# kouyt5/lightning-asr

Hardware: AMD Instinct MI355X
Metric: audio-seconds/sec training (asr13x1, bs=32, 10 s clips) (higher is better)
Workload: dtype bf16; 1 GPU; asr13x1 QuartzNet-CTC train step, bs=32/GPU, 10 s synthetic 16 kHz clips, labels.txt vocab (C=28), HIP mel+conv+CTC+NovoGrad, random-init weights; global_batch=32, n_class=28, parallelism=dp1, feature_prefetch=True, hip_graph=True, staged_backward=False

## Files before the change

### include/lasr.h

```cpp
#ifndef LASR_H
#define LASR_H

#include <stddef.h>
#include <stdint.h>

#ifdef __cplusplus
extern "C" {
#endif

#define LASR_VERSION 108

enum { LASR_F32 = 0, LASR_BF16 = 1 };
enum { LASR_ACT_NONE = 0, LASR_ACT_RELU = 1, LASR_ACT_SWISH = 2 };
enum { LASR_VARIANT_PLAIN = 0, LASR_VARIANT_CONTEXT = 1, LASR_VARIANT_CONTEXT_SE = 2 };
enum {
  LASR_E_ARG = -1,
  LASR_E_SHAPE = -2,
  LASR_E_WORKSPACE = -3,
  LASR_E_FORMAT = -4,
  LASR_E_UNSUPPORTED = -5,
  LASR_E_IO = -6
};

int lasr_version(void);
// ... 75 lines not shown
int lasr_bn_finalize(const float* stats, const float* gamma, const float* beta, float* running_mean,
                     float* running_var, float* coef, float* saved, int64_t C, int64_t n_rows, float eps,
                     float momentum, int training, void* stream);
typedef struct {
  const float* gamma; const float* beta; const float* running_mean; const float* running_var; float* coef; int64_t C;
} lasr_bn_eval_desc;
int lasr_bn_eval_coef_many(const lasr_bn_eval_desc* descs, int n_descs, float eps, void* stream);

typedef struct {
  const float* partials; int n_partials;
  const float* gamma; const float* beta; float* running_mean; float* running_var;
  float* coef; float* saved; float* stats;
} lasr_bn_branch;
int lasr_bn_finalize_partials(const lasr_bn_branch* branches, int n_branches, int64_t C, int64_t n_rows, float eps,
                              float momentum, void* stream);

typedef struct { const uint64_t* step; uint64_t seed; uint32_t unit; float p; } lasr_dropout;
int lasr_mask_lengths_step(const float* pct, int64_t B, int64_t T, int32_t* lens, uint64_t* step_counter, void* stream);
int lasr_dropout_mask(const lasr_dropout* dropout, int64_t n, uint8_t* keep, void* stream);
int lasr_bn_act_fwd_drop(const void* y, const float* coef, const void* y2, const float* coef2, const float* se_scale, void* out,
                         int dtype, int64_t B, int64_t T, int64_t C, int act, const lasr_dropout* dropout, void* stream);
int lasr_bn_act_bwd_stats_drop(const void* dout, const void* y, const float* coef, const float* saved, const void* y2,
                               const float* coef2, const float* saved2, const float* se_scale, const float* se_grad, float* sums,
                               float* sums2, int dtype, int64_t B, int64_t T, int64_t C, int act, const lasr_dropout* dropout,
                               void* workspace, size_t workspace_bytes, void* stream);
int lasr_se_bwd_drop(const void* dout, const void* y, const float* coef, const void* y2, const float* coef2, const float* scale,
                     const float* hidden, const float* pooled, const float* W1, const float* W2, int dtype, int64_t B, int64_t T,
                     int64_t C, int act, const lasr_dropout* dropout, float* seg, float* dW1, float* dW2, void* workspace,
                     size_t workspace_bytes, void* stream);
size_t lasr_bn_se_bwd_workspace_bytes(int64_t B, int64_t T, int64_t C);
// ... 248 lines not shown
```

### lightning_asr_amd/_lib.py

```python
from __future__ import annotations

import ctypes as C
import os

_HERE = os.path.dirname(os.path.abspath(__file__))
LIB_PATH = os.environ.get("LASR_LIB_PATH", os.path.join(_HERE, "liblasr.so"))

F32, BF16 = 0, 1
ACT_NONE, ACT_RELU, ACT_SWISH = 0, 1, 2
LEN_LEAD = 1 << 30
VARIANT = {"plain": 0, "context": 1, "context_se": 2}

_p, _i64, _i32, _f32, _sz = C.c_void_p, C.c_int64, C.c_int, C.c_float, C.c_size_t


class Dropout(C.Structure):
    _fields_ = [("step", C.c_void_p), ("seed", C.c_uint64), ("unit", C.c_uint32), ("p", C.c_float)]


class WaveSrc(C.Structure):
    _fields_ = [("wave", C.c_void_p), ("wave_dtype", C.c_int32), ("dither", C.c_void_p), ("dither_seed", C.c_uint64),
                ("dither_step", C.c_void_p), ("pitch", C.c_int64)]


# ... 29 lines not shown
    "lasr_gemm_batch": (_i32, [_p, _i32, _i32, _i32, _i32, _i32, _i32, _p, _sz, _p]),
    "lasr_bn_finalize": (_i32, [_p, _p, _p, _p, _p, _p, _p, _i64, _i64, _f32, _f32, _i32, _p]),
    "lasr_bn_eval_coef_many": (_i32, [_p, _i32, _f32, _p]),
    "lasr_bn_act_fwd": (_i32, [_p, _p, _p, _p, _p, _p, _i32, _i64, _i64, _i64, _i32, _p]),
    "lasr_bn_bwd_workspace_bytes": (_sz, [_i64, _i64, _i64]),
    "lasr_bn_act_bwd_stats": (_i32, [_p] * 11 + [_i32, _i64, _i64, _i64, _i32, _p, _sz, _p]),
    "lasr_bn_act_bwd_apply": (_i32, [_p] * 20 + [_i32, _i64, _i64, _i64, _i32, _p, _sz, _p]),
    "lasr_bn_bwd_apply_workspace_bytes": (_sz, [_i64]),
    "lasr_reduce_many": (_i32, [_p, _i32, _p]),
    "lasr_gemm_batch_split_partials": (_i32, [_p, _i32, _i32, _i32, _i32, _i32, _p, _sz, _p, _p, _p]),
    "lasr_gemm_multi_split_partials": (_i32, [_p, _i32, _i32, _p, _p, _p]),
    "lasr_dwconv_wgrad_partials": (_i32, [_p, _p, _i32, _i64, _i64, _i64, _i32, _i32, _p, _sz, _p, _p]),
    "lasr_dwconv_bwd_fused": (_i32, [_p, _p, _p, _p, _p, _i32, _i64, _i64, _i64, _i32, _p, _sz, _p, _p]),
    "lasr_gemm_batch_partials": (_i32, [_p, _i32, _i32, _i32, _i32, _i32, _p, _sz, _p, _p, _p]),
    "lasr_bn_finalize_partials": (_i32, [_p, _i32, _i64, _i64, C.c_float, C.c_float, _p]),
    "lasr_seqsum": (_i32, [_p, _i32, _i64, _i64, _i64, _p, _p]),
    "lasr_se_fwd": (_i32, [_p, _p, _p, _p, _i64, _i64, _i64, _p, _p, _p, _p]),
    "lasr_se_bwd_workspace_bytes": (_sz, [_i64, _i64]),
    "lasr_se_bwd": (_i32, [_p] * 10 + [_i32, _i64, _i64, _i64, _i32, _p, _p, _p, _p, _sz, _p]),
    "lasr_bilstm_saved_bytes": (_sz, [_i64, _i64]),
    "lasr_bilstm_fwd": (_i32, [_p] * 9 + [_i64, _i64, _p, _i32, _i64, _i64, _p, _p]),
    "lasr_bilstm_bwd_workspace_bytes": (_sz, [_i64]),
    "lasr_bilstm_bwd": (_i32, [_p, _i32, _i64, _i64, _p, _p, _p, _i64, _i64, _p, _p, _p, _p, _p, _p, _sz, _p]),
    "lasr_copy_cols": (_i32, [_p, _i32, _i64, _i64, _p, _i32, _i64, _i64, _i64, _i64, _i32, _p]),
    "lasr_log_softmax": (_i32, [_p, _p, _p, _i64, _i64, _p]),
    "lasr_log_softmax_bwd": (_i32, [_p, _p, _p, _i64, _i64, _p]),
    "lasr_ctc_workspace_bytes": (_sz, [_i64, _i64, _i64]),
    "lasr_ctc_loss": (_i32, [_p, _p, _p, _p, _i64, _i64, _i64, _i64, _i32, _p, _p, _p, _p, _sz, _p]),
    "lasr_ctc_loss_mel": (_i32, [_p, _p, _p, _p, _i64, _i64, _i64, _i64, _i32, _p, _p, _p, _p, _sz,
                                 _p, _p, _p, _p, _i64, _i64, _i32, _p, _p, _i32, _p, _p, _p, _sz, _p]),
# ... 126 lines not shown
```

### lightning_asr_amd/csrc/conv.hip

```cpp
#include "common.h"
#include "fused.h"

namespace lasr {

static thread_local const DwTapCtx* g_dw_tap_ctx = nullptr;
void dw_taps_set_ctx(const DwTapCtx* ctx) { g_dw_tap_ctx = ctx; }
bool dw_taps_enabled() {
  static const bool on = !(getenv("LASR_DW_TAPS") && atoi(getenv("LASR_DW_TAPS")) == 0);
  return on;
}
const uint32_t* dw_taps_for(const float* w, int flip, int64_t C) {
  (void)flip;
  const DwTapCtx* c = g_dw_tap_ctx;
  if (!c || C % 64 != 0) return nullptr;
  for (int i = 0; i < c->n; ++i)
    if (c->w[i] == w && c->C[i] == (int)C) return c->t[i];
  return nullptr;
}

static constexpr int kCB = 64;
static constexpr int kTT = 128;
static constexpr int kR = 8;
static constexpr int kMaxK = 128;

// ... 422 lines not shown
namespace dwm {
static constexpr int TT = 512;
static constexpr int KWMAX = 128;
static constexpr int TIN = TT - 16 + KWMAX;
static constexpr int LDI = 1296;
static constexpr int RS = 128;
static constexpr int LDST = 160;
static constexpr int IMG_BYTES = kCB * LDI;
static constexpr int STAGE_BYTES = RS * LDST;
static constexpr int WROW = 160;
static constexpr int WSM_OFF = IMG_BYTES + STAGE_BYTES;
static constexpr int SMEM = WSM_OFF + kCB * WROW * 4;
static_assert(LDI >= TIN * 2 && LDI % 16 == 0, "image pitch");
}
struct DwBnIn {
  const bf16_t* y; const bf16_t* y2; const float* coef; const float* coef2; bf16_t* out; int act;
};
typedef __bf16 dw_bf16x8 __attribute__((ext_vector_type(8)));
typedef float dw_f32x4 __attribute__((ext_vector_type(4)));
typedef short dw_s16x4 __attribute__((ext_vector_type(4)));

#ifdef LASR_DW_STAMPS
__device__ unsigned long long* g_dw_stamps = nullptr;
#define DW_STAMP(i_) do { if (g_dw_stamps && threadIdx.x == 0) g_dw_stamps[(blockIdx.y * gridDim.x + blockIdx.x) * 8 + (i_)] = wall_clock64(); } while (0)
#else
#define DW_STAMP(i_) do {} while (0)
#endif
template <int NKS, int NSET, bool FUSE = false>
__device__ __forceinline__ void dwconv_s1_mfma_body(const bf16_t* __restrict__ x, const float* __restrict__ w,
                                                    const bf16_t* __restrict__ addend, bf16_t* __restrict__ y,
                                                    int Tlen, int C, int k, int flip, int bx, int by, int bz, int gz,
                                                    char* smem_raw, const uint32_t* __restrict__ taps, const DwBnIn bn = DwBnIn{}) {
  using namespace dwm;
  char* img = smem_raw;
  char* stage = smem_raw + IMG_BYTES;
  uint32_t* wsm = reinterpret_cast<uint32_t*>(smem_raw + WSM_OFF);
  const int tid = threadIdx.x, lane = tid & 63, wid = tid >> 6;
  const int b = by, c0 = bx * kCB;
  if (taps) {
    static_assert(WROW == kDwTapRow, "tap table row");
    const uint4* src = reinterpret_cast<const uint4*>(taps + ((size_t)flip * C + c0) * WROW);
    uint4 tv[kCB * WROW / 4 / 512];
#pragma unroll
    for (int it = 0; it < kCB * WROW / 4 / 512; ++it) tv[it] = src[tid + 512 * it];
#pragma unroll
    for (int it = 0; it < kCB * WROW / 4 / 512; ++it) reinterpret_cast<uint4*>(wsm)[tid + 512 * it] = tv[it];
  } else {
    constexpr int kIt = kCB * WROW / 512;
    float f0[kIt], f1[kIt];
#pragma unroll
    for (int it = 0; it < kIt; ++it) {
      const int i = tid + 512 * it;
      const int ch = i / WROW, idx = i - ch * WROW;
      const int i0 = idx < 80 ? 2 * idx : 2 * (idx - 80) + 1;
      const int j0 = i0 - 24, j1 = i0 - 23;
      const float* wc = w + (size_t)min(c0 + ch, C - 1) * k;
      const bool cok = c0 + ch < C;
      const int q0 = min(max(j0, 0), k - 1), q1 = min(max(j1, 0), k - 1);
      const float a0 = wc[flip ? k - 1 - q0 : q0], a1 = wc[flip ? k - 1 - q1 : q1];
      f0[it] = __uint_as_float(__float_as_uint(a0) & ((cok && j0 >= 0 && j0 < k) ? 0xffffffffu : 0u));
      f1[it] = __uint_as_float(__float_as_uint(a1) & ((cok && j1 >= 0 && j1 < k) ? 0xffffffffu : 0u));
    }
    __builtin_amdgcn_sched_barrier(0);
#pragma unroll
    for (int it = 0; it < kIt; ++it) wsm[tid + 512 * it] = (uint32_t)f32_to_bf16(f0[it]) | ((uint32_t)f32_to_bf16(f1[it]) << 16);
  }
  const int pad = k / 2, P = (pad + 7) & ~7, sh = P - pad;
  constexpr int KW = 32 * NKS;
  const bf16_t* xb = FUSE ? nullptr : x + (size_t)b * Tlen * C;
  const int n16 = lane & 15, g4 = lane >> 4;
  float ca[8], cb[8], ca2[8], cb2[8];
  if (FUSE) {
    const int ccl = min(c0 + ((tid & 7) << 3), C - 8);
    auto ld8 = [](const float* p, float (&o)[8]) {
      const float4 u = *reinterpret_cast<const float4*>(p), q = *reinterpret_cast<const float4*>(p + 4);
      o[0] = u.x; o[1] = u.y; o[2] = u.z; o[3] = u.w; o[4] = q.x; o[5] = q.y; o[6] = q.z; o[7] = q.w;
    };
    ld8(bn.coef + ccl, ca); ld8(bn.coef + C + ccl, cb);
    if (bn.y2) { ld8(bn.coef2 + ccl, ca2); ld8(bn.coef2 + C + ccl, cb2); }
  }

  DW_STAMP(0);
  constexpr int TTS = 256 * NSET;
  for (int tA = bz * TTS; tA < Tlen; tA += TTS * gz) {
    const int tin = TTS - 16 + KW;
    constexpr int kRounds = (TTS - 16 + KWMAX + RS - 1) / RS;
    uint4 v[kRounds][2];
    if (!FUSE) {
#pragma unroll
      for (int r = 0; r < kRounds; ++r) {
#pragma unroll
        for (int h = 0; h < 2; ++h) {
          const int ch = tid + 512 * h;
          const int tau = r * RS + (ch >> 3);
          const int t = tA - P + tau;
          const int cc = c0 + ((ch & 7) << 3);
// ... 900 lines not shown
    with_dtype(dtype, [&](auto t) {
      rc = with_int<4, 8>(small ? 4 : 8, [&](auto r) {
        using T = typename decltype(t)::type;
        launch_lds(dwconv_fwd_kernel<T, decltype(r)::value>, g2, dim3(256), shmem, st, (const T*)x, w, (const T*)addend, (T*)y, Tin, Tout, C, k,
                   stride, flip);
      });
    });
  }
  prof_end(tok, st);
  LASR_TRY(rc);
  LASR_LAUNCH_CHECK("dwconv_fwd_kernel");
  return 0;
}

int lasr::dwconv_fwd_bn(const void* y, const float* coef, const void* y2, const float* coef2, int act, const float* w, void* out, void* u,
                        int64_t B, int64_t T, int64_t C, int k, void* stream) {
  LASR_CHECK_ARG(y && coef && w && out && u && (!y2 || coef2), "dwconv_fwd_bn: null pointer");
  if (k < 1 || k > kMaxK || !(k & 1) || C < 8 || T <= 0 || B <= 0 || B >= 65536) return 1;
  const DwShape s = dw_shape(B, T, C, k, LASR_BF16, al16(y) && al16(y2) && al16(out) && al16(u) && al16(coef) && al16(coef2));
  static const bool full_too = getenv("LASR_BN_DW_FUSE") && atoi(getenv("LASR_BN_DW_FUSE")) == 2;
  if (!s.fwd || (s.nset == 2 && !full_too)) return 1;
  const dim3 gridm((unsigned)cdiv(C, kCB), (unsigned)B, (unsigned)s.gz_d);
  DwBnIn bn;
  bn.y = (const bf16_t*)y; bn.y2 = (const bf16_t*)y2; bn.coef = coef; bn.coef2 = coef2; bn.out = (bf16_t*)out; bn.act = act;
  hipStream_t st = as_stream(stream);
  const int tok = prof_begin(LASR_PROF_DWCONV, st, 2.0 * (double)B * T * C * k, (double)B * T * C * (y2 ? 4 : 3) * 2);
  const uint32_t* taps = dw_taps_for(w, 0, C);
  const int rc = with_dw_tile(s, [&](auto nks, auto nset) {
    launch_lds(dwconv_s1_mfma_bn_kernel<nks.value, nset.value>, gridm, dim3(512), dwm::SMEM, st, bn, w, (bf16_t*)u, (int)T, (int)C, k, taps);
  });
  prof_end(tok, st);
  LASR_TRY(rc);
  LASR_LAUNCH_CHECK("dwconv_s1_mfma_bn_kernel");
  return 0;
}

extern "C" size_t lasr_dwconv_wgrad_workspace_bytes(int64_t B, int64_t Tout, int64_t C, int k) {
  return (size_t)B * cdiv(Tout, kWChunkG) * C * k * sizeof(float);
}
// ... 138 lines not shown
```

### lightning_asr_amd/csrc/fused.h

```cpp
#pragma once
#include "common.h"

namespace lasr {

int dwconv_fwd_bn(const void* y, const float* coef, const void* y2, const float* coef2, int act, const float* w, void* out, void* u,
                  int64_t B, int64_t T, int64_t C, int k, void* stream);

static constexpr int kDwTapRow = 160;
struct DwTapJobs {
  int n; int blk0[17]; const float* w[16]; uint32_t* out[16]; int C[16]; int k[16];
};
__device__ __forceinline__ uint32_t dw_tap_entry(const float* __restrict__ w, int C, int k, int e) {
  const int flip = e / (C * kDwTapRow), r = e - flip * (C * kDwTapRow);
  const int c = r / kDwTapRow, idx = r - c * kDwTapRow;
  const int i0 = idx < kDwTapRow / 2 ? 2 * idx : 2 * (idx - kDwTapRow / 2) + 1;
  const int j0 = i0 - 24, j1 = i0 - 23;
  const float* wc = w + (size_t)c * k;
  const int q0 = min(max(j0, 0), k - 1), q1 = min(max(j1, 0), k - 1);
  const float a0 = wc[flip ? k - 1 - q0 : q0], a1 = wc[flip ? k - 1 - q1 : q1];
  const uint32_t m0 = (j0 >= 0 && j0 < k) ? 0xffffffffu : 0u, m1 = (j1 >= 0 && j1 < k) ? 0xffffffffu : 0u;
  return (uint32_t)f32_to_bf16(__uint_as_float(__float_as_uint(a0) & m0)) | ((uint32_t)f32_to_bf16(__uint_as_float(__float_as_uint(a1) & m1)) << 16);
}
struct DwTapCtx { int n; const float* w[16]; const uint32_t* t[16]; int C[16]; };
void dw_taps_set_ctx(const DwTapCtx* ctx);
// ... 17 lines not shown
```

### lightning_asr_amd/csrc/model.hip

```cpp
#include "common.h"
#include "mel.h"
#include "fused.h"
#include "gemm.h"
#include "lstm_body.h"
#include "se_seqsum.h"
#include <string>
#include <vector>
#include <math.h>

namespace lasr {

static constexpr float kBnEps = 1e-3f;
static constexpr float kBnMom = 0.1f;

struct TensorInfo {
  std::string name;
  int64_t shape[4] = {0, 0, 0, 0};
  int ndim = 0;
  int kind = 0;
  int64_t offset = 0;
  int64_t numel = 1;
};

struct BnRef { int64_t gamma = -1, beta = -1, rmean = -1, rvar = -1; };
// ... 467 lines not shown
    for (size_t i = 0; i < descs.size(); i += 64)
      LASR_TRY(lasr_bn_eval_coef_many(descs.data() + i, (int)std::min<size_t>(64, descs.size() - i), kBnEps, stream));
    if (eval_fold(m->cfg.dtype)) {
      std::vector<lasr_fold_desc> fd;
      for (const Unit& u : m->units)
        if (fold_unit(u))
          fd.push_back({params + u.w_pw, params + u.w_res, atf(ws, u.o_coef), atf(ws, u.o_coef2), at(ws, u.o_wfold), atf(ws, u.o_bfold), u.co, u.ci});
      for (size_t i = 0; i < fd.size(); i += 32)
        LASR_TRY(lasr_fold_bn_weights_many(fd.data() + i, (int)std::min<size_t>(32, fd.size() - i), stream));
    }
  }
  const void* x = feats;
  int64_t Tx = T_in;
  static const bool bn_dw_fuse = !(getenv("LASR_BN_DW_FUSE") && atoi(getenv("LASR_BN_DW_FUSE")) == 0);
  const Unit* pend = nullptr;
  auto bn_act_of = [&](const Unit& v) -> int {
    ProfScope ps_bn(LASR_PROF_BN, stream, (double)N * v.co * dtype_size(dt) * (v.has_res ? 3 : 2));
    const lasr_dropout drop = {m->drop_step, m->drop_seed, (uint32_t)(&v - m->units.data()), dropping ? m->drop_p : 0.f};
    return lasr_bn_act_fwd_drop(at(ws, v.o_y), atf(ws, v.o_coef), v.has_res ? at(ws, v.o_y2) : nullptr,
                                v.has_res ? atf(ws, v.o_coef2) : nullptr, v.has_se ? atf(ws, v.o_se_scale) : nullptr, at(ws, v.o_out), dt, B,
                                T, v.co, v.act ? m->cfg.act : LASR_ACT_NONE, dropping ? &drop : nullptr, stream);
  };
  RoctxRange rr_fwd(training ? "lasr:forward (training)" : "lasr:forward (eval)");
  for (size_t ui = 0; ui < m->units.size(); ++ui) {
    const Unit& u = m->units[ui];
    RoctxRange rr_unit(u.rx_fwd.c_str());
    if (pend && !(u.has_dw && u.stride == 1 && !u.ctx_before)) {
      LASR_TRY(bn_act_of(*pend));
      pend = nullptr;
    }
    if (u.ctx_before) {
      {
// ... 1 lines not shown
        for (int d = 0; d < 2; ++d) pr[d] = {x, wptr(m, params, ws, m->lstm.w_ih[d]), atf(ws, p.o_gx[d]), N, 160, 256, nullptr, nullptr, 0, nullptr};
        LASR_TRY(lasr_gemm_batch(pr, 2, dt, LASR_F32, 0, 0, 1, scratch, p.scratch_bytes, stream));
      }
      LASR_TRY(lasr_copy_cols(x, dt, 256, 0, at(ws, p.o_cat), dt, 336, 0, N, 256, 0, stream));
      LASR_TRY(lasr_bilstm_fwd(atf(ws, p.o_gx[0]), atf(ws, p.o_gx[1]), params + m->lstm.w_hh[0], params + m->lstm.w_hh[1],
                               params + m->lstm.b_ih[0], params + m->lstm.b_hh[0], params + m->lstm.b_ih[1], params + m->lstm.b_hh[1],
                               lens, B, T, at(ws, p.o_cat), dt, 336, 256, atf(ws, p.o_lstm_saved), stream));
      x = at(ws, p.o_cat);
    }
    const void* gin = x;
    if (u.has_dw) {
      int fused = 1;
      if (pend) {
        fused = dwconv_fwd_bn(at(ws, pend->o_y), atf(ws, pend->o_coef), pend->has_res ? at(ws, pend->o_y2) : nullptr,
                              pend->has_res ? atf(ws, pend->o_coef2) : nullptr, pend->act ? m->cfg.act : LASR_ACT_NONE, params + u.w_dw,
                              at(ws, pend->o_out), at(ws, u.o_u), B, T, u.ci, u.k, stream);
        if (fused < 0) return fused;
        if (fused == 1) LASR_TRY(bn_act_of(*pend));
        pend = nullptr;
      }
      if (fused == 1) LASR_TRY(lasr_dwconv_fwd(x, params + u.w_dw, nullptr, at(ws, u.o_u), dt, B, Tx, u.ci, u.k, u.stride, 0, stream));
      gin = at(ws, u.o_u);
    }
    if (!training && eval_fold(dt) && fold_unit(u)) {
      LASR_TRY(lasr_gemm_dual(gin, u.ci, x, u.ci, at(ws, u.o_wfold), atf(ws, u.o_bfold), at(ws, u.o_out), N, u.co, u.masked ? lens : nullptr,
                              T, u.act ? m->cfg.act : LASR_ACT_NONE, stream));
      x = at(ws, u.o_out);
      Tx = T;
      continue;
    }
    float* stats = training ? atf(ws, u.o_stats) : nullptr;
    float* stats2 = (training && u.has_res) ? atf(ws, u.o_stats2) : nullptr;
// ... 1 lines not shown
    {
      lasr_gemm_problem pr[2];
      pr[0] = {gin, wptr(m, params, ws, u.w_pw), at(ws, u.o_y), N, u.co, u.ci, nullptr, u.masked ? lens : nullptr, T, stats};
      if (u.has_res) pr[1] = {x, wptr(m, params, ws, u.w_res), at(ws, u.o_y2), N, u.co, u.ci, nullptr, nullptr, 0, stats2};
      const int np = u.has_res ? 2 : 1;
      if (training && !no_fuse()) {
        const float* parts[2] = {nullptr, nullptr};
        int tiles[2] = {0, 0};
        LASR_TRY(lasr_gemm_batch_partials(pr, np, dt, dt, 0, 0, scratch, p.scratch_bytes, parts, tiles, stream));
        lasr_bn_branch br[2];
        br[0] = {parts[0], tiles[0], params + u.bn.gamma, params + u.bn.beta, buffers + u.bn.rmean, buffers + u.bn.rvar,
                 atf(ws, u.o_coef), atf(ws, u.o_saved), stats};
        if (u.has_res)
          br[1] = {parts[1], tiles[1], params + u.bn_res.gamma, params + u.bn_res.beta, buffers + u.bn_res.rmean,
                   buffers + u.bn_res.rvar, atf(ws, u.o_coef2), atf(ws, u.o_saved2), stats2};
        ProfScope ps(LASR_PROF_BN, stream, 0.0);
        int merged = 1;
        if (u.has_se) {
          merged = bn_finalize_partials_seqsum(br, np, u.co, N, kBnEps, kBnMom, at(ws, u.o_y), dt, B, T, atf(ws, u.o_se_sum), stream);
          if (merged < 0 || merged > 1) return merged;
          se_sums_done = merged == 0;
        }
        if (merged == 1) LASR_TRY(lasr_bn_finalize_partials(br, np, u.co, N, kBnEps, kBnMom, stream));
      } else {
        LASR_TRY(lasr_gemm_batch(pr, np, dt, dt, 0, 0, 1, scratch, p.scratch_bytes, stream));
        if (training) {
          LASR_TRY(lasr_bn_finalize(stats, params + u.bn.gamma, params + u.bn.beta, buffers + u.bn.rmean, buffers + u.bn.rvar,
                                    atf(ws, u.o_coef), atf(ws, u.o_saved), u.co, N, kBnEps, kBnMom, training, stream));
          if (u.has_res)
            LASR_TRY(lasr_bn_finalize(stats2, params + u.bn_res.gamma, params + u.bn_res.beta, buffers + u.bn_res.rmean,
                                      buffers + u.bn_res.rvar, atf(ws, u.o_coef2), atf(ws, u.o_saved2), u.co, N, kBnEps, kBnMom,
                                      training, stream));
        }
      }
    }
    bool se_applied = false;
    if (u.has_se) {
      ProfScope ps_se(LASR_PROF_BN, stream, (double)N * u.co * dtype_size(dt));
// ... 395 lines not shown
```

### lightning_asr_amd/csrc/norm.hip

```cpp
#include "common.h"
#include "reduce_body.h"
#include "se_seqsum.h"
#include "fused.h"
#include "dropout.h"
#include <algorithm>
#include <string.h>

namespace lasr {

template <typename T, bool TO_BTC>
__global__ __launch_bounds__(256) void transpose_kernel(const void* __restrict__ in_, void* __restrict__ out_,
                                                        int64_t C, int64_t Tt) {
  __shared__ float tile[32][33];
  const int b = blockIdx.z;
  const int64_t c0 = (int64_t)blockIdx.y * 32, t0 = (int64_t)blockIdx.x * 32;
  const int tx = threadIdx.x & 31, ty = threadIdx.x >> 5;
  if (TO_BTC) {
    const float* in = reinterpret_cast<const float*>(in_) + (int64_t)b * C * Tt;
    T* out = reinterpret_cast<T*>(out_) + (int64_t)b * C * Tt;
    for (int i = ty; i < 32; i += 8)
      if (c0 + i < C && t0 + tx < Tt) tile[i][tx] = in[(c0 + i) * Tt + t0 + tx];
    __syncthreads();
    for (int i = ty; i < 32; i += 8)
      if (t0 + i < Tt && c0 + tx < C) Elem<T>::st(out + (t0 + i) * C + c0 + tx, tile[tx][i]);
// ... 32 lines not shown
    return;
  }
  const int64_t n4 = n >> 2;
  const int64_t stride = (int64_t)cast_blocks * 256;
  for (int64_t e = blockIdx.x * (int64_t)256 + threadIdx.x; e < n4; e += stride) {
    const float4 v = reinterpret_cast<const float4*>(in)[e];
    uint2 o;
    o.x = (uint32_t)f32_to_bf16(v.x) | ((uint32_t)f32_to_bf16(v.y) << 16);
    o.y = (uint32_t)f32_to_bf16(v.z) | ((uint32_t)f32_to_bf16(v.w) << 16);
    reinterpret_cast<uint2*>(out)[e] = o;
  }
  if (blockIdx.x == 0)
    for (int64_t e = (n4 << 2) + threadIdx.x; e < n; e += 256) out[e] = f32_to_bf16(in[e]);
}

__device__ __forceinline__ void bn_finalize_channel(float s, float q, int64_t c, const float* __restrict__ gamma,
                                                    const float* __restrict__ beta, float* __restrict__ rmean,
                                                    float* __restrict__ rvar, float* __restrict__ coef, float* __restrict__ saved,
                                                    int64_t C, float n, float eps, float momentum, int training) {
  float mean, var;
  if (training) {
    const double m = (double)s / n;
    double v = (double)q / n - m * m;
    if (v < 0) v = 0;
    mean = (float)m;
    var = (float)v;
    if (rmean) {
      rmean[c] = (1.f - momentum) * rmean[c] + momentum * mean;
      const float unbiased = n > 1.f ? (float)(v * (double)n / ((double)n - 1.0)) : var;
      rvar[c] = (1.f - momentum) * rvar[c] + momentum * unbiased;
    }
  } else {
    mean = rmean[c];
    var = rvar[c];
  }
  const float rstd = 1.0f / sqrtf(var + eps);
  const float a = gamma[c] * rstd;
  coef[c] = a;
  coef[C + c] = beta[c] - mean * a;
  if (saved) { saved[c] = mean; saved[C + c] = rstd; }
}

__global__ void bn_finalize_kernel(const float* __restrict__ stats, const float* __restrict__ gamma,
                                   const float* __restrict__ beta, float* __restrict__ rmean, float* __restrict__ rvar,
                                   float* __restrict__ coef, float* __restrict__ saved, int64_t C, float n, float eps,
                                   float momentum, int training) {
  const int64_t c = blockIdx.x * (int64_t)blockDim.x + threadIdx.x;
  if (c >= C) return;
  bn_finalize_channel(training ? stats[c] : 0.f, training ? stats[C + c] : 0.f, c, gamma, beta, rmean, rvar, coef, saved, C, n, eps,
                      momentum, training);
}

struct BnEvalMany { lasr_bn_eval_desc d[64]; };
__global__ __launch_bounds__(256) void bn_eval_coef_many_kernel(BnEvalMany a, float eps) {
  const lasr_bn_eval_desc q = a.d[blockIdx.y];
  const int64_t c = blockIdx.x * (int64_t)blockDim.x + threadIdx.x;
  if (c >= q.C) return;
  bn_finalize_channel(0.f, 0.f, c, q.gamma, q.beta, const_cast<float*>(q.running_mean), const_cast<float*>(q.running_var), q.coef, nullptr,
                      q.C, 1.f, eps, 0.f, 0);
}

template <int LANES = 8>
__device__ __forceinline__ double partial_lane_sum(const float* __restrict__ partials, int n_part, int64_t ncols, int64_t c, int pl) {
  double a0 = 0.0, a1 = 0.0, a2 = 0.0, a3 = 0.0;
  for (int p = pl; p < n_part; p += 16 * LANES) {
    float v[16];
#pragma unroll
    for (int i = 0; i < 16; ++i) {
      const int r = p + LANES * i;
      const float x = partials[(int64_t)min(r, n_part - 1) * ncols + c];
      v[i] = r < n_part ? x : 0.f;
    }
#pragma unroll
    for (int i = 0; i < 16; i += 4) {
      a0 += (double)v[i]; a1 += (double)v[i + 1]; a2 += (double)v[i + 2]; a3 += (double)v[i + 3];
    }
  }
  return (a0 + a1) + (a2 + a3);
}

__global__ __launch_bounds__(256) void reduce_partials_kernel(const float* __restrict__ partials, int n_part, int64_t ncols,
                                                              float* __restrict__ out0, int64_t split, float* __restrict__ out1) {
  __shared__ double s_acc[8][33];
  const int cl = threadIdx.x & 31, pl = threadIdx.x >> 5;
  const int64_t c = (int64_t)blockIdx.x * 32 + cl;
  s_acc[pl][cl] = c < ncols ? partial_lane_sum(partials, n_part, ncols, c, pl) : 0.0;
  __syncthreads();
  if (pl == 0 && c < ncols) {
    double s = 0.0;
#pragma unroll
    for (int i = 0; i < 8; ++i) s += s_acc[i][cl];
    if (c < split) out0[c] = (float)s;
    else if (out1) out1[c - split] = (float)s;
  }
}

struct BnBranch {
  const float* partials; int n_part;
  const float* gamma; const float* beta; float* rmean; float* rvar; float* coef; float* saved; float* stats;
};
struct BnBranch2 { BnBranch b[2]; };

__global__ __launch_bounds__(256) void bn_finalize_partials_kernel(BnBranch2 br, int64_t C, float n, float eps, float momentum) {
  __shared__ double s_acc[8][33];
  const BnBranch& b = blockIdx.y ? br.b[1] : br.b[0];
  const int cl = threadIdx.x & 31, pl = threadIdx.x >> 5;
  const int64_t c = (int64_t)blockIdx.x * 16 + (cl & 15);
  s_acc[pl][cl] = c < C ? partial_lane_sum(b.partials, b.n_part, 2 * C, (int64_t)(cl >> 4) * C + c, pl) : 0.0;
  __syncthreads();
  if (pl == 0 && cl < 16 && c < C) {
    double s = 0.0, q = 0.0;
#pragma unroll
    for (int i = 0; i < 8; ++i) { s += s_acc[i][cl]; q += s_acc[i][16 + cl]; }
    if (b.stats) { b.stats[c] = (float)s; b.stats[C + c] = (float)q; }
    bn_finalize_channel((float)s, (float)q, c, b.gamma, b.beta, b.rmean, b.rvar, b.coef, b.saved, C, n, eps, momentum, 1);
  }
// ... 585 lines not shown
        const float d1 = SE ? fmaf(d[j], sev[j], sgv[j]) : d[j];
        o1[j] = masked ? 0.f : fmaf(G[j], d1, fmaf(Bc[j], yv[j], Cc[j]));
      }
      if (live) Vec<bf16_t>::store(dy + off[u], o1);
      if (HAS2) {
        lds_vec8(&s_tab[7][cl * V], G); lds_vec8(&s_tab[8][cl * V], Bc); lds_vec8(&s_tab[9][cl * V], Cc);
#pragma unroll
        for (int j = 0; j < V; ++j) o2[j] = fmaf(G[j], d[j], fmaf(Bc[j], rv[j], Cc[j]));
        if (live) Vec<bf16_t>::store(dy2 + off[u], o2);
      }
    }
  }
  });
}

static int bn_sliced_rpc(int dtype, int64_t rows, int64_t C, bool se, bool drop, int per_utt, bool reduced_sums) {
  static const int target = getenv("LASR_BN_SLICED") ? atoi(getenv("LASR_BN_SLICED")) : 256;
  if (target <= 0 || dtype != LASR_BF16 || se || drop || per_utt || reduced_sums || C % kSlCh != 0 || rows < 4096) return 0;
  const int64_t slices = C / kSlCh;
  const int64_t nchunk = std::max<int64_t>(1, std::min<int64_t>(target / slices, rows / kSlLanes));
  return (int)cdiv(rows, nchunk);
}

}

using namespace lasr;

extern "C" int lasr_bn_act_bwd_stats_drop(const void* dout, const void* y, const float* coef, const float* saved, const void* y2,
                                          const float* coef2, const float* saved2, const float* se_scale, const float* se_grad,
                                          float* sums, float* sums2, int dtype, int64_t B, int64_t T_, int64_t C, int act,
// ... 140 lines not shown
  const DropArgs da = make_drop(dropout);
  const int64_t rows = B * T_;
  const size_t shmem = (size_t)4 * C * sizeof(float);
  with_bn_variant(dtype, y2 != nullptr, se_scale != nullptr, da.step != nullptr, [&](auto t, auto h2, auto se, auto drop) {
    using T = typename decltype(t)::type;
    hipLaunchKernelGGL((bn_act_fwd_kernel<T, h2.value, se.value, drop.value>), dim3((unsigned)cdiv(rows, kFwdSlabRows)), dim3(256), shmem,
                       as_stream(stream), (const T*)y, coef, (const T*)y2, coef2, se_scale, (T*)out, (int)rows, (int)T_, (int)C, act, da);
  });
  LASR_LAUNCH_CHECK("bn_act_fwd_kernel");
  return 0;
}

extern "C" int lasr_bn_act_fwd(const void* y, const float* coef, const void* y2, const float* coef2, const float* se_scale,
                               void* out, int dtype, int64_t B, int64_t T_, int64_t C, int act, void* stream) {
  return lasr_bn_act_fwd_drop(y, coef, y2, coef2, se_scale, out, dtype, B, T_, C, act, nullptr, stream);
}

extern "C" size_t lasr_bn_bwd_workspace_bytes(int64_t B, int64_t T_, int64_t C) {
  return (size_t)cdiv(B * T_, kRowsPerBlock) * 4 * C * sizeof(float) + (size_t)10 * C * sizeof(float);
}

extern "C" int lasr_bn_act_bwd_stats(const void* dout, const void* y, const float* coef, const float* saved, const void* y2,
                                     const float* coef2, const float* saved2, const float* se_scale, const float* se_grad,
                                     float* sums, float* sums2, int dtype, int64_t B, int64_t T_, int64_t C, int act,
                                     void* workspace, size_t workspace_bytes, void* stream) {
  return lasr_bn_act_bwd_stats_drop(dout, y, coef, saved, y2, coef2, saved2, se_scale, se_grad, sums, sums2, dtype, B, T_, C, act, nullptr,
                                    workspace, workspace_bytes, stream);
}

extern "C" int lasr_bn_act_bwd_stats_drop(const void* dout, const void* y, const float* coef, const float* saved, const void* y2,
// ... 395 lines not shown
```

Baseline: 157,000 audio-seconds/sec.

## Fold BN partial-stat finalize into consumer forward kernels

Instead of launching a separate BN finalize kernel after each conv's partial statistics, the finalize is deferred and done redundantly per channel slice inside the consumer kernel: either the fused depthwise-conv+BN kernel or a new sliced BN-activation forward kernel. One designated block writes running stats, coef and saved values. This removes a kernel launch and a dependency bubble per BN layer. The cost is that every block re-reduces the partials, and the finalize arithmetic is reworked with fma and contract-off updates, which may change numerics slightly. It is enabled by default for bf16, non-SE, non-dropout units with C a multiple of 64.

New measurement: 158,600 audio-seconds/sec, median of 6. 1.1% higher.

```diff
diff --git a/include/lasr.h b/include/lasr.h
--- a/include/lasr.h
+++ b/include/lasr.h
@@ -113,6 +113,8 @@
 } lasr_bn_branch;
 int lasr_bn_finalize_partials(const lasr_bn_branch* branches, int n_branches, int64_t C, int64_t n_rows, float eps,
                               float momentum, void* stream);
+int lasr_bn_act_fwd_partials(const lasr_bn_branch* branches, int n_branches, float eps, float momentum, const void* y,
+                             const void* y2, void* out, int dtype, int64_t B, int64_t T, int64_t C, int act, void* stream);
 
 typedef struct { const uint64_t* step; uint64_t seed; uint32_t unit; float p; } lasr_dropout;
 int lasr_mask_lengths_step(const float* pct, int64_t B, int64_t T, int32_t* lens, uint64_t* step_counter, void* stream);
diff --git a/lightning_asr_amd/_lib.py b/lightning_asr_amd/_lib.py
--- a/lightning_asr_amd/_lib.py
+++ b/lightning_asr_amd/_lib.py
@@ -67,6 +67,7 @@
     "lasr_dwconv_bwd_fused": (_i32, [_p, _p, _p, _p, _p, _i32, _i64, _i64, _i64, _i32, _p, _sz, _p, _p]),
     "lasr_gemm_batch_partials": (_i32, [_p, _i32, _i32, _i32, _i32, _i32, _p, _sz, _p, _p, _p]),
     "lasr_bn_finalize_partials": (_i32, [_p, _i32, _i64, _i64, C.c_float, C.c_float, _p]),
+    "lasr_bn_act_fwd_partials": (_i32, [_p, _i32, C.c_float, C.c_float, _p, _p, _p, _i32, _i64, _i64, _i64, _i32, _p]),
     "lasr_seqsum": (_i32, [_p, _i32, _i64, _i64, _i64, _p, _p]),
     "lasr_se_fwd": (_i32, [_p, _p, _p, _p, _i64, _i64, _i64, _p, _p, _p, _p]),
     "lasr_se_bwd_workspace_bytes": (_sz, [_i64, _i64]),
diff --git a/lightning_asr_amd/csrc/bn_slice.h b/lightning_asr_amd/csrc/bn_slice.h
--- /dev/null
+++ b/lightning_asr_amd/csrc/bn_slice.h
@@ -0,0 +1,152 @@
+#pragma once
+#include "common.h"
+
+namespace lasr {
+
+__device__ __forceinline__ void bn_finalize_channel(float s, float q, int64_t c, const float* __restrict__ gamma,
+                                                    const float* __restrict__ beta, float* __restrict__ rmean,
+                                                    float* __restrict__ rvar, float* __restrict__ coef, float* __restrict__ saved,
+                                                    int64_t C, float n, float eps, float momentum, int training) {
+  float mean, var;
+  if (training) {
+    const double m = (double)s / n;
+    double v = fma(-m, m, (double)q / n);
+    if (v < 0) v = 0;
+    mean = (float)m;
+    var = (float)v;
+    if (rmean) {
+#pragma clang fp contract(off)
+      const float keep = 1.f - momentum;
+      const float km = keep * rmean[c], nm = momentum * mean;
+      rmean[c] = km + nm;
+      const float unbiased = n > 1.f ? (float)(v * (double)n / ((double)n - 1.0)) : var;
+      const float kv = keep * rvar[c], nv = momentum * unbiased;
+      rvar[c] = kv + nv;
+    }
+  } else {
+    mean = rmean[c];
+    var = rvar[c];
+  }
+  const float rstd = 1.0f / sqrtf(var + eps);
+  const float a = gamma[c] * rstd;
+  coef[c] = a;
+  coef[C + c] = fmaf(-a, mean, beta[c]);
+  if (saved) { saved[c] = mean; saved[C + c] = rstd; }
+}
+
+template <int LANES = 8>
+__device__ __forceinline__ double partial_lane_sum(const float* __restrict__ partials, int n_part, int64_t ncols, int64_t c, int pl) {
+  double a0 = 0.0, a1 = 0.0, a2 = 0.0, a3 = 0.0;
+  for (int p = pl; p < n_part; p += 16 * LANES) {
+    float v[16];
+#pragma unroll
+    for (int i = 0; i < 16; ++i) {
+      const int r = p + LANES * i;
+      const float x = partials[(int64_t)min(r, n_part - 1) * ncols + c];
+      v[i] = r < n_part ? x : 0.f;
+    }
+#pragma unroll
+    for (int i = 0; i < 16; i += 4) {
+      a0 += (double)v[i]; a1 += (double)v[i + 1]; a2 += (double)v[i + 2]; a3 += (double)v[i + 3];
+    }
+  }
+  return (a0 + a1) + (a2 + a3);
+}
+
+template <int NC>
+__device__ __forceinline__ void partial_lane_sum_cols(const float* const (&col)[NC], int n_part, int64_t ncols, int pl, double (&out)[NC]) {
+  double a[NC][4];
+#pragma unroll
+  for (int k = 0; k < NC; ++k) a[k][0] = a[k][1] = a[k][2] = a[k][3] = 0.0;
+  for (int p = pl; p < n_part; p += 16 * 8) {
+    float v[NC][16];
+#pragma unroll
+    for (int i = 0; i < 16; ++i) {
+      const int r = p + 8 * i;
+      const int64_t ro = (int64_t)min(r, n_part - 1) * ncols;
+#pragma unroll
+      for (int k = 0; k < NC; ++k) {
+        const float x = col[k][ro];
+        v[k][i] = r < n_part ? x : 0.f;
+      }
+    }
+#pragma unroll
+    for (int k = 0; k < NC; ++k)
+#pragma unroll
+      for (int i = 0; i < 16; i += 4) {
+        a[k][0] += (double)v[k][i]; a[k][1] += (double)v[k][i + 1]; a[k][2] += (double)v[k][i + 2]; a[k][3] += (double)v[k][i + 3];
+      }
+  }
+#pragma unroll
+  for (int k = 0; k < NC; ++k) out[k] = (a[k][0] + a[k][1]) + (a[k][2] + a[k][3]);
+}
+
+struct BnBranch {
+  const float* partials; int n_part;
+  const float* gamma; const float* beta; float* rmean; float* rvar; float* coef; float* saved; float* stats;
+};
+struct BnBranch2 { BnBranch b[2]; };
+
+struct BnSliceIn { BnBranch2 br; int nb; float n, eps, momentum; };
+
+static constexpr int kBnSliceCh = 64;
+static constexpr int kBnSliceAccBytes = 8 * 4 * kBnSliceCh * 8;
+static constexpr int kBnSliceTabFloats = 2 * 4 * kBnSliceCh;
+
+template <bool HAS2>
+__device__ __forceinline__ void bn_slice_finalize(const BnSliceIn& in, int C, int c0, bool writer, double* __restrict__ s_acc,
+                                                  float* __restrict__ s_tab) {
+  constexpr int NB = HAS2 ? 2 : 1;
+  const int tid = threadIdx.x, ch = tid & 63, pl = tid >> 6;
+  const BnBranch& b0 = in.br.b[0];
+  const BnBranch& b1 = in.br.b[1];
+  const bool fin = tid < NB * kBnSliceCh;
+  const bool second = HAS2 && __builtin_amdgcn_readfirstlane(pl) == 1;
+  const int cf = c0 + ch;
+  const float* gp = second ? b1.gamma : b0.gamma;
+  const float* bp = second ? b1.beta : b0.beta;
+  float* rmean = second ? b1.rmean : b0.rmean;
+  float* rvar = second ? b1.rvar : b0.rvar;
+  float* coef = second ? b1.coef : b0.coef;
+  float* saved = second ? b1.saved : b0.saved;
+  float* stats = second ? b1.stats : b0.stats;
+  float g = gp[cf], be = bp[cf], rm = (rmean ? rmean : gp)[cf], rv = (rmean ? rvar : gp)[cf];
+  const int64_t nc = 2 * (int64_t)C;
+  if (HAS2 && b0.n_part == b1.n_part) {
+    const float* const col[4] = {b0.partials + cf, b0.partials + C + cf, b1.partials + cf, b1.partials + C + cf};
+    double o[4];
+    partial_lane_sum_cols<4>(col, b0.n_part, nc, pl, o);
+#pragma unroll
+    for (int k = 0; k < 4; ++k) s_acc[(pl * 4 + k) * kBnSliceCh + ch] = o[k];
+  } else {
+#pragma unroll
+    for (int j = 0; j < NB; ++j) {
+      const BnBranch& b = j ? b1 : b0;
+      const float* const col[2] = {b.partials + cf, b.partials + C + cf};
+      double o[2];
+      partial_lane_sum_cols<2>(col, b.n_part, nc, pl, o);
+      s_acc[(pl * 4 + 2 * j) * kBnSliceCh + ch] = o[0];
+      s_acc[(pl * 4 + 2 * j + 1) * kBnSliceCh + ch] = o[1];
+    }
+  }
+  __syncthreads();
+  if (fin) {
+    const int j = pl;
+    double s = 0.0, q = 0.0;
+#pragma unroll
+    for (int i = 0; i < 8; ++i) { s += s_acc[(i * 4 + 2 * j) * kBnSliceCh + ch]; q += s_acc[(i * 4 + 2 * j + 1) * kBnSliceCh + ch]; }
+    float* tab = s_tab + j * 4 * kBnSliceCh;
+    const bool upd = writer && rmean;
+    bn_finalize_channel((float)s, (float)q, 0, &g, &be, upd ? &rm : nullptr, upd ? &rv : nullptr, tab + ch, tab + 2 * kBnSliceCh + ch,
+                        kBnSliceCh, in.n, in.eps, in.momentum, 1);
+    if (writer) {
+      if (stats) { stats[cf] = (float)s; stats[C + cf] = (float)q; }
+      if (upd) { rmean[cf] = rm; rvar[cf] = rv; }
+      coef[cf] = tab[ch]; coef[C + cf] = tab[kBnSliceCh + ch];
+      if (saved) { saved[cf] = tab[2 * kBnSliceCh + ch]; saved[C + cf] = tab[3 * kBnSliceCh + ch]; }
+    }
+  }
+  __syncthreads();
+}
+
+}
diff --git a/lightning_asr_amd/csrc/conv.hip b/lightning_asr_amd/csrc/conv.hip
--- a/lightning_asr_amd/csrc/conv.hip
+++ b/lightning_asr_amd/csrc/conv.hip
@@ -1,5 +1,6 @@
 #include "common.h"
 #include "fused.h"
+#include "bn_slice.h"
 
 namespace lasr {
 
@@ -460,7 +461,7 @@
 static_assert(LDI >= TIN * 2 && LDI % 16 == 0, "image pitch");
 }
 struct DwBnIn {
-  const bf16_t* y; const bf16_t* y2; const float* coef; const float* coef2; bf16_t* out; int act;
+  const bf16_t* y; const bf16_t* y2; const float* coef; const float* coef2; bf16_t* out; int act; BnSliceIn fin;
 };
 typedef __bf16 dw_bf16x8 __attribute__((ext_vector_type(8)));
 typedef float dw_f32x4 __attribute__((ext_vector_type(4)));
@@ -483,14 +484,37 @@
   uint32_t* wsm = reinterpret_cast<uint32_t*>(smem_raw + WSM_OFF);
   const int tid = threadIdx.x, lane = tid & 63, wid = tid >> 6;
   const int b = by, c0 = bx * kCB;
+  float ca[8], cb[8], ca2[8], cb2[8];
+  auto bn_coefs = [&]() {
+  if (FUSE) {
+    const int ccl = min(c0 + ((tid & 7) << 3), C - 8);
+    auto ld8 = [](const float* p, float (&o)[8]) {
+      const float4 u = *reinterpret_cast<const float4*>(p), q = *reinterpret_cast<const float4*>(p + 4);
+      o[0] = u.x; o[1] = u.y; o[2] = u.z; o[3] = u.w; o[4] = q.x; o[5] = q.y; o[6] = q.z; o[7] = q.w;
+    };
+    if (bn.fin.nb) {
+      double* s_acc = reinterpret_cast<double*>(img);
+      float* s_tab = reinterpret_cast<float*>(img + kBnSliceAccBytes);
+      const bool writer = by == 0 && bz == 0;
+      if (bn.y2) bn_slice_finalize<true>(bn.fin, C, c0, writer, s_acc, s_tab);
+      else bn_slice_finalize<false>(bn.fin, C, c0, writer, s_acc, s_tab);
+      const int o8 = (tid & 7) << 3;
+      ld8(s_tab + o8, ca); ld8(s_tab + kBnSliceCh + o8, cb);
+      if (bn.y2) { ld8(s_tab + 4 * kBnSliceCh + o8, ca2); ld8(s_tab + 5 * kBnSliceCh + o8, cb2); }
+    } else {
+      ld8(bn.coef + ccl, ca); ld8(bn.coef + C + ccl, cb);
+      if (bn.y2) { ld8(bn.coef2 + ccl, ca2); ld8(bn.coef2 + C + ccl, cb2); }
+    }
+  }
+  };
   if (taps) {
     static_assert(WROW == kDwTapRow, "tap table row");
     const uint4* src = reinterpret_cast<const uint4*>(taps + ((size_t)flip * C + c0) * WROW);
-    uint4 tv[kCB * WROW / 4 / 512];
-#pragma unroll
-    for (int it = 0; it < kCB * WROW / 4 / 512; ++it) tv[it] = src[tid + 512 * it];
-#pragma unroll
-    for (int it = 0; it < kCB * WROW / 4 / 512; ++it) reinterpret_cast<uint4*>(wsm)[tid + 512 * it] = tv[it];
+    static_assert(kCB * WROW / 4 / 512 == 5, "tap table chunks per thread");
+    const uint4 tv0 = src[tid], tv1 = src[tid + 512], tv2 = src[tid + 1024], tv3 = src[tid + 1536], tv4 = src[tid + 2048];
+    bn_coefs();
+    uint4* wd = reinterpret_cast<uint4*>(wsm);
+    wd[tid] = tv0; wd[tid + 512] = tv1; wd[tid + 1024] = tv2; wd[tid + 1536] = tv3; wd[tid + 2048] = tv4;
   } else {
     constexpr int kIt = kCB * WROW / 512;
     float f0[kIt], f1[kIt];
@@ -510,22 +534,12 @@
     __builtin_amdgcn_sched_barrier(0);
 #pragma unroll
     for (int it = 0; it < kIt; ++it) wsm[tid + 512 * it] = (uint32_t)f32_to_bf16(f0[it]) | ((uint32_t)f32_to_bf16(f1[it]) << 16);
+    bn_coefs();
   }
   const int pad = k / 2, P = (pad + 7) & ~7, sh = P - pad;
   constexpr int KW = 32 * NKS;
   const bf16_t* xb = FUSE ? nullptr : x + (size_t)b * Tlen * C;
   const int n16 = lane & 15, g4 = lane >> 4;
-  float ca[8], cb[8], ca2[8], cb2[8];
-  if (FUSE) {
-    const int ccl = min(c0 + ((tid & 7) << 3), C - 8);
-    auto ld8 = [](const float* p, float (&o)[8]) {
-      const float4 u = *reinterpret_cast<const float4*>(p), q = *reinterpret_cast<const float4*>(p + 4);
-      o[0] = u.x; o[1] = u.y; o[2] = u.z; o[3] = u.w; o[4] = q.x; o[5] = q.y; o[6] = q.z; o[7] = q.w;
-    };
-    ld8(bn.coef + ccl, ca); ld8(bn.coef + C + ccl, cb);
-    if (bn.y2) { ld8(bn.coef2 + ccl, ca2); ld8(bn.coef2 + C + ccl, cb2); }
-  }
-
   DW_STAMP(0);
   constexpr int TTS = 256 * NSET;
   for (int tA = bz * TTS; tA < Tlen; tA += TTS * gz) {
@@ -1456,8 +1470,9 @@
 }
 
 int lasr::dwconv_fwd_bn(const void* y, const float* coef, const void* y2, const float* coef2, int act, const float* w, void* out, void* u,
-                        int64_t B, int64_t T, int64_t C, int k, void* stream) {
+                        int64_t B, int64_t T, int64_t C, int k, void* stream, const lasr_bn_branch* partials_of, float eps, float momentum) {
   LASR_CHECK_ARG(y && coef && w && out && u && (!y2 || coef2), "dwconv_fwd_bn: null pointer");
+  LASR_CHECK_SHAPE(!partials_of || C % kCB == 0, "dwconv_fwd_bn: a consumer-side finalize needs C=%lld a multiple of 64", (long long)C);
   if (k < 1 || k > kMaxK || !(k & 1) || C < 8 || T <= 0 || B <= 0 || B >= 65536) return 1;
   const DwShape s = dw_shape(B, T, C, k, LASR_BF16, al16(y) && al16(y2) && al16(out) && al16(u) && al16(coef) && al16(coef2));
   static const bool full_too = getenv("LASR_BN_DW_FUSE") && atoi(getenv("LASR_BN_DW_FUSE")) == 2;
@@ -1465,6 +1480,8 @@
   const dim3 gridm((unsigned)cdiv(C, kCB), (unsigned)B, (unsigned)s.gz_d);
   DwBnIn bn;
   bn.y = (const bf16_t*)y; bn.y2 = (const bf16_t*)y2; bn.coef = coef; bn.coef2 = coef2; bn.out = (bf16_t*)out; bn.act = act;
+  memset(&bn.fin, 0, sizeof(bn.fin));
+  if (partials_of) LASR_TRY(bn_slice_in(partials_of, y2 ? 2 : 1, B * T, eps, momentum, &bn.fin));
   hipStream_t st = as_stream(stream);
   const int tok = prof_begin(LASR_PROF_DWCONV, st, 2.0 * (double)B * T * C * k, (double)B * T * C * (y2 ? 4 : 3) * 2);
   const uint32_t* taps = dw_taps_for(w, 0, C);
diff --git a/lightning_asr_amd/csrc/fused.h b/lightning_asr_amd/csrc/fused.h
--- a/lightning_asr_amd/csrc/fused.h
+++ b/lightning_asr_amd/csrc/fused.h
@@ -4,7 +4,10 @@
 namespace lasr {
 
 int dwconv_fwd_bn(const void* y, const float* coef, const void* y2, const float* coef2, int act, const float* w, void* out, void* u,
-                  int64_t B, int64_t T, int64_t C, int k, void* stream);
+                  int64_t B, int64_t T, int64_t C, int k, void* stream, const lasr_bn_branch* partials_of = nullptr, float eps = 0.f,
+                  float momentum = 0.f);
+struct BnSliceIn;
+int bn_slice_in(const lasr_bn_branch* branches, int n_branches, int64_t n_rows, float eps, float momentum, BnSliceIn* in);
 
 static constexpr int kDwTapRow = 160;
 struct DwTapJobs {
diff --git a/lightning_asr_amd/csrc/model.hip b/lightning_asr_amd/csrc/model.hip
--- a/lightning_asr_amd/csrc/model.hip
+++ b/lightning_asr_amd/csrc/model.hip
@@ -505,8 +505,16 @@
   int64_t Tx = T_in;
   static const bool bn_dw_fuse = !(getenv("LASR_BN_DW_FUSE") && atoi(getenv("LASR_BN_DW_FUSE")) == 0);
   const Unit* pend = nullptr;
+  static const bool bn_fwd_finalize = !(getenv("LASR_BN_FWD_FINALIZE") && atoi(getenv("LASR_BN_FWD_FINALIZE")) == 0);
+  const Unit* owed = nullptr;
+  lasr_bn_branch owed_br[2];
   auto bn_act_of = [&](const Unit& v) -> int {
     ProfScope ps_bn(LASR_PROF_BN, stream, (double)N * v.co * dtype_size(dt) * (v.has_res ? 3 : 2));
+    if (owed == &v) {
+      owed = nullptr;
+      return lasr_bn_act_fwd_partials(owed_br, v.has_res ? 2 : 1, kBnEps, kBnMom, at(ws, v.o_y), v.has_res ? at(ws, v.o_y2) : nullptr,
+                                      at(ws, v.o_out), dt, B, T, v.co, v.act ? m->cfg.act : LASR_ACT_NONE, stream);
+    }
     const lasr_dropout drop = {m->drop_step, m->drop_seed, (uint32_t)(&v - m->units.data()), dropping ? m->drop_p : 0.f};
     return lasr_bn_act_fwd_drop(at(ws, v.o_y), atf(ws, v.o_coef), v.has_res ? at(ws, v.o_y2) : nullptr,
                                 v.has_res ? atf(ws, v.o_coef2) : nullptr, v.has_se ? atf(ws, v.o_se_scale) : nullptr, at(ws, v.o_out), dt, B,
@@ -538,8 +546,9 @@
       if (pend) {
         fused = dwconv_fwd_bn(at(ws, pend->o_y), atf(ws, pend->o_coef), pend->has_res ? at(ws, pend->o_y2) : nullptr,
                               pend->has_res ? atf(ws, pend->o_coef2) : nullptr, pend->act ? m->cfg.act : LASR_ACT_NONE, params + u.w_dw,
-                              at(ws, pend->o_out), at(ws, u.o_u), B, T, u.ci, u.k, stream);
+                              at(ws, pend->o_out), at(ws, u.o_u), B, T, u.ci, u.k, stream, owed == pend ? owed_br : nullptr, kBnEps, kBnMom);
         if (fused < 0) return fused;
+        if (fused == 0) owed = nullptr;
         if (fused == 1) LASR_TRY(bn_act_of(*pend));
         pend = nullptr;
       }
@@ -571,14 +580,20 @@
         if (u.has_res)
           br[1] = {parts[1], tiles[1], params + u.bn_res.gamma, params + u.bn_res.beta, buffers + u.bn_res.rmean,
                    buffers + u.bn_res.rvar, atf(ws, u.o_coef2), atf(ws, u.o_saved2), stats2};
-        ProfScope ps(LASR_PROF_BN, stream, 0.0);
-        int merged = 1;
-        if (u.has_se) {
-          merged = bn_finalize_partials_seqsum(br, np, u.co, N, kBnEps, kBnMom, at(ws, u.o_y), dt, B, T, atf(ws, u.o_se_sum), stream);
-          if (merged < 0 || merged > 1) return merged;
-          se_sums_done = merged == 0;
+        if (bn_fwd_finalize && dt == LASR_BF16 && !u.has_se && !dropping && u.co % 64 == 0) {
+          owed = &u;
+          owed_br[0] = br[0];
+          owed_br[1] = br[u.has_res ? 1 : 0];
+        } else {
+          ProfScope ps(LASR_PROF_BN, stream, 0.0);
+          int merged = 1;
+          if (u.has_se) {
+            merged = bn_finalize_partials_seqsum(br, np, u.co, N, kBnEps, kBnMom, at(ws, u.o_y), dt, B, T, atf(ws, u.o_se_sum), stream);
+            if (merged < 0 || merged > 1) return merged;
+            se_sums_done = merged == 0;
+          }
+          if (merged == 1) LASR_TRY(lasr_bn_finalize_partials(br, np, u.co, N, kBnEps, kBnMom, stream));
         }
-        if (merged == 1) LASR_TRY(lasr_bn_finalize_partials(br, np, u.co, N, kBnEps, kBnMom, stream));
       } else {
         LASR_TRY(lasr_gemm_batch(pr, np, dt, dt, 0, 0, 1, scratch, p.scratch_bytes, stream));
         if (training) {
diff --git a/lightning_asr_amd/csrc/norm.hip b/lightning_asr_amd/csrc/norm.hip
--- a/lightning_asr_amd/csrc/norm.hip
+++ b/lightning_asr_amd/csrc/norm.hip
@@ -2,6 +2,7 @@
 #include "reduce_body.h"
 #include "se_seqsum.h"
 #include "fused.h"
+#include "bn_slice.h"
 #include "dropout.h"
 #include <algorithm>
 #include <string.h>
@@ -70,33 +71,6 @@
     for (int64_t e = (n4 << 2) + threadIdx.x; e < n; e += 256) out[e] = f32_to_bf16(in[e]);
 }
 
-__device__ __forceinline__ void bn_finalize_channel(float s, float q, int64_t c, const float* __restrict__ gamma,
-                                                    const float* __restrict__ beta, float* __restrict__ rmean,
-                                                    float* __restrict__ rvar, float* __restrict__ coef, float* __restrict__ saved,
-                                                    int64_t C, float n, float eps, float momentum, int training) {
-  float mean, var;
-  if (training) {
-    const double m = (double)s / n;
-    double v = (double)q / n - m * m;
-    if (v < 0) v = 0;
-    mean = (float)m;
-    var = (float)v;
-    if (rmean) {
-      rmean[c] = (1.f - momentum) * rmean[c] + momentum * mean;
-      const float unbiased = n > 1.f ? (float)(v * (double)n / ((double)n - 1.0)) : var;
-      rvar[c] = (1.f - momentum) * rvar[c] + momentum * unbiased;
-    }
-  } else {
-    mean = rmean[c];
-    var = rvar[c];
-  }
-  const float rstd = 1.0f / sqrtf(var + eps);
-  const float a = gamma[c] * rstd;
-  coef[c] = a;
-  coef[C + c] = beta[c] - mean * a;
-  if (saved) { saved[c] = mean; saved[C + c] = rstd; }
-}
-
 __global__ void bn_finalize_kernel(const float* __restrict__ stats, const float* __restrict__ gamma,
                                    const float* __restrict__ beta, float* __restrict__ rmean, float* __restrict__ rvar,
                                    float* __restrict__ coef, float* __restrict__ saved, int64_t C, float n, float eps,
@@ -114,25 +88,6 @@
   if (c >= q.C) return;
   bn_finalize_channel(0.f, 0.f, c, q.gamma, q.beta, const_cast<float*>(q.running_mean), const_cast<float*>(q.running_var), q.coef, nullptr,
                       q.C, 1.f, eps, 0.f, 0);
-}
-
-template <int LANES = 8>
-__device__ __forceinline__ double partial_lane_sum(const float* __restrict__ partials, int n_part, int64_t ncols, int64_t c, int pl) {
-  double a0 = 0.0, a1 = 0.0, a2 = 0.0, a3 = 0.0;
-  for (int p = pl; p < n_part; p += 16 * LANES) {
-    float v[16];
-#pragma unroll
-    for (int i = 0; i < 16; ++i) {
-      const int r = p + LANES * i;
-      const float x = partials[(int64_t)min(r, n_part - 1) * ncols + c];
-      v[i] = r < n_part ? x : 0.f;
-    }
-#pragma unroll
-    for (int i = 0; i < 16; i += 4) {
-      a0 += (double)v[i]; a1 += (double)v[i + 1]; a2 += (double)v[i + 2]; a3 += (double)v[i + 3];
-    }
-  }
-  return (a0 + a1) + (a2 + a3);
 }
 
 __global__ __launch_bounds__(256) void reduce_partials_kernel(const float* __restrict__ partials, int n_part, int64_t ncols,
@@ -150,12 +105,6 @@
     else if (out1) out1[c - split] = (float)s;
   }
 }
-
-struct BnBranch {
-  const float* partials; int n_part;
-  const float* gamma; const float* beta; float* rmean; float* rvar; float* coef; float* saved; float* stats;
-};
-struct BnBranch2 { BnBranch b[2]; };
 
 __global__ __launch_bounds__(256) void bn_finalize_partials_kernel(BnBranch2 br, int64_t C, float n, float eps, float momentum) {
   __shared__ double s_acc[8][33];
@@ -771,6 +720,68 @@
   });
 }
 
+template <bool HAS2, int RB = 4, int WPE = HAS2 ? 2 : 4>
+__global__ __launch_bounds__(512, WPE) void bn_act_fwd_sliced_kernel(const bf16_t* __restrict__ y, const bf16_t* __restrict__ y2, BnSliceIn in,
+                                                                   bf16_t* __restrict__ out, int rows, int C, int act_rt, int rpc) {
+  __shared__ double s_acc[kBnSliceAccBytes / 8];
+  __shared__ __attribute__((aligned(16))) float s_tab[kBnSliceTabFloats];
+  constexpr int V = 8;
+  const int tid = threadIdx.x, cl = tid & 7, rl = tid >> 3;
+  const int c0 = blockIdx.x * kSlCh, c = c0 + cl * V;
+  const int r0 = blockIdx.y * rpc, r1 = min(r0 + rpc, rows);
+  uint4 ry[RB], rr[RB];
+  auto load_rows = [&](int base, uint4 (&dy_)[RB], uint4 (&dr_)[RB]) {
+#pragma unroll
+    for (int u = 0; u < RB; ++u) {
+      const uint32_t off = (uint32_t)min(base + rl + u * kSlLanes, rows - 1) * (uint32_t)C + (uint32_t)c;
+      dy_[u] = Vec<bf16_t>::raw(y + off);
+      if (HAS2) dr_[u] = Vec<bf16_t>::raw(y2 + off);
+    }
+  };
+  load_rows(r0, ry, rr);
+  bn_slice_finalize<HAS2>(in, C, c0, blockIdx.y == 0, s_acc, s_tab);
+  float a[V], b[V], a2[V], b2[V];
+  lds_vec8(s_tab + cl * V, a); lds_vec8(s_tab + kBnSliceCh + cl * V, b);
+  if (HAS2) { lds_vec8(s_tab + 4 * kBnSliceCh + cl * V, a2); lds_vec8(s_tab + 5 * kBnSliceCh + cl * V, b2); }
+  with_act(act_rt, [&](auto act_c) {
+  constexpr int act = decltype(act_c)::value;
+  for (int base = r0;;) {
+    const int nbase = base + RB * kSlLanes;
+    const bool more = nbase < r1;
+    uint4 ny[RB], nr[RB];
+    if (more) load_rows(nbase, ny, nr);
+#pragma unroll
+    for (int u = 0; u < RB; ++u) {
+      const int r = base + rl + u * kSlLanes;
+      float v[V], w[V], o[V];
+      Vec<bf16_t>::unpack(ry[u], v);
+#pragma unroll
+      for (int j = 0; j < V; ++j) o[j] = fmaf(v[j], a[j], b[j]);
+      if (HAS2) {
+        Vec<bf16_t>::unpack(rr[u], w);
+#pragma unroll
+        for (int j = 0; j < V; ++j) o[j] += fmaf(w[j], a2[j], b2[j]);
+      }
+#pragma unroll
+      for (int j = 0; j < V; ++j) o[j] = act_fwd(o[j], act);
+      if (r < r1) Vec<bf16_t>::store(out + (uint32_t)r * (uint32_t)C + (uint32_t)c, o);
+    }
+    if (!more) break;
+#pragma unroll
+    for (int u = 0; u < RB; ++u) { ry[u] = ny[u]; if (HAS2) rr[u] = nr[u]; }
+    base = nbase;
+  }
+  });
+}
+
+static int bn_fwd_sliced_rpc(int64_t rows, int64_t C) {
+  static const int forced = getenv("LASR_BN_FWD_SLICED") ? atoi(getenv("LASR_BN_FWD_SLICED")) : 0;
+  const int target = forced > 0 ? forced : 256;
+  const int64_t slices = C / kSlCh;
+  const int64_t nchunk = std::max<int64_t>(1, std::min<int64_t>(target / slices, rows / kSlLanes));
+  return (int)cdiv(rows, nchunk);
+}
+
 static int bn_sliced_rpc(int dtype, int64_t rows, int64_t C, bool se, bool drop, int per_utt, bool reduced_sums) {
   static const int target = getenv("LASR_BN_SLICED") ? atoi(getenv("LASR_BN_SLICED")) : 256;
   if (target <= 0 || dtype != LASR_BF16 || se || drop || per_utt || reduced_sums || C % kSlCh != 0 || rows < 4096) return 0;
@@ -941,6 +952,38 @@
 extern "C" int lasr_bn_act_fwd(const void* y, const float* coef, const void* y2, const float* coef2, const float* se_scale,
                                void* out, int dtype, int64_t B, int64_t T_, int64_t C, int act, void* stream) {
   return lasr_bn_act_fwd_drop(y, coef, y2, coef2, se_scale, out, dtype, B, T_, C, act, nullptr, stream);
+}
+
+int lasr::bn_slice_in(const lasr_bn_branch* branches, int n_branches, int64_t n_rows, float eps, float momentum, BnSliceIn* in) {
+  LASR_CHECK_ARG(branches && (n_branches == 1 || n_branches == 2) && n_rows > 0 && in, "bn_slice_in: bad argument");
+  for (int i = 0; i < 2; ++i) {
+    const lasr_bn_branch& q = branches[i < n_branches ? i : 0];
+    LASR_CHECK_ARG(q.partials && q.n_partials > 0 && q.gamma && q.beta && q.coef && (!q.running_mean || q.running_var),
+                   "bn_slice_in: null pointer");
+    in->br.b[i] = {q.partials, q.n_partials, q.gamma, q.beta, q.running_mean, q.running_var, q.coef, q.saved, q.stats};
+  }
+  in->nb = n_branches; in->n = (float)n_rows; in->eps = eps; in->momentum = momentum;
+  return 0;
+}
+
+extern "C" int lasr_bn_act_fwd_partials(const lasr_bn_branch* branches, int n_branches, float eps, float momentum, const void* y,
+                                        const void* y2, void* out, int dtype, int64_t B, int64_t T_, int64_t C, int act, void* stream) {
+  LASR_CHECK_ARG(y && out && n_branches == (y2 ? 2 : 1), "lasr_bn_act_fwd_partials: bad argument");
+  LASR_TRY(check_bn_shape("lasr_bn_act_fwd_partials", dtype, B, T_, C));
+  LASR_CHECK_SHAPE(dtype == LASR_BF16 && C % kSlCh == 0, "lasr_bn_act_fwd_partials: bf16 and C=%lld a multiple of 64 only", (long long)C);
+  LASR_CHECK_ARG(reinterpret_cast<uintptr_t>(y) % 16 == 0 && reinterpret_cast<uintptr_t>(y2) % 16 == 0 && reinterpret_cast<uintptr_t>(out) % 16 == 0,
+                 "lasr_bn_act_fwd_partials: 16-byte alignment");
+  const int64_t rows = B * T_;
+  BnSliceIn in;
+  LASR_TRY(bn_slice_in(branches, n_branches, rows, eps, momentum, &in));
+  const int rpc = bn_fwd_sliced_rpc(rows, C);
+  const dim3 grid((unsigned)(C / kSlCh), (unsigned)cdiv(rows, rpc));
+  with_bool(y2 != nullptr, [&](auto h2) {
+    hipLaunchKernelGGL((bn_act_fwd_sliced_kernel<decltype(h2)::value>), grid, dim3(kSlThreads), 0, as_stream(stream), (const bf16_t*)y,
+                       (const bf16_t*)y2, in, (bf16_t*)out, (int)rows, (int)C, act, rpc);
+  });
+  LASR_LAUNCH_CHECK("bn_act_fwd_sliced_kernel");
+  return 0;
 }
 
 extern "C" size_t lasr_bn_bwd_workspace_bytes(int64_t B, int64_t T_, int64_t C) {
```
